# puzzlepaint/camera_calibration

Hardware: NVIDIA H100
Metric: LM iterations/sec (higher is better)
Workload: dtype f64

## Files before the change

camera_calibration_b200/csrc/ba_dense.cu:

```cuda

#include <algorithm>
#include <cstdio>

#include "ba_kernels.h"
#include "ba_tile.cuh"

namespace b200ba {

namespace {

constexpr int BM = 128;
constexpr int LDT = BM + 4;
__host__ __device__ constexpr int gemm_threads(int bn) { return 4 * (bn / 32) * 32; }
constexpr size_t gemm_smem(int bn, int bk, int stages) {
  return static_cast<size_t>(stages) * bk * (LDT + bn + 4) * sizeof(double);
}

__device__ __forceinline__ void cp_async16(void* smem, const void* gmem, int src_bytes) {
  const unsigned s = static_cast<unsigned>(__cvta_generic_to_shared(smem));
  asm volatile("cp.async.cg.shared.global [%0], [%1], 16, %2;\n" ::"r"(s), "l"(gmem), "r"(src_bytes));
}
__device__ __forceinline__ void cp_async8(void* smem, const void* gmem, int src_bytes) {
  const unsigned s = static_cast<unsigned>(__cvta_generic_to_shared(smem));
  asm volatile("cp.async.ca.shared.global [%0], [%1], 8, %2;\n" ::"r"(s), "l"(gmem), "r"(src_bytes));
// ... 23 lines not shown

  __device__ __forceinline__ void init(const double* __restrict__ X, int64_t ldx, int rows, int i0, bool al) {
    aligned = al;
    int i;
    if (al) {
      kk0 = threadIdx.x / CH;
      const int ch = threadIdx.x % CH;
      i = i0 + 2 * ch;
      off0 = kk0 * LD + 2 * ch;
      bytes = (i + 1 < rows) ? 16 : ((i < rows) ? 8 : 0);
    } else {
      kk0 = threadIdx.x / W;
      const int ii = threadIdx.x % W;
      i = i0 + ii;
      off0 = kk0 * LD + ii;
      bytes = (i < rows) ? 8 : 0;
    }
    src = X + static_cast<int64_t>(kk0) * ldx + min(i, max(rows - 1, 0));
  }
  __device__ __forceinline__ void issue(double* dst, int k0, int K, const double* __restrict__ X, int64_t ldx) {
    const double* p = src;
    if (aligned) {
#pragma unroll
      for (int q = 0; q < Q16; ++q) {
        const int nb = (k0 + kk0 + q * KS16 < K) ? bytes : 0;
        cp_async16(dst + off0 + q * KS16 * LD, nb ? p : X, nb);
        p += KS16 * ldx;
      }
    } else {
#pragma unroll
      for (int q = 0; q < Q8; ++q) {
        const int nb = (k0 + kk0 + q * KS8 < K) ? bytes : 0;
        cp_async8(dst + off0 + q * KS8 * LD, nb ? p : X, nb);
        p += KS8 * ldx;
      }
    }
    src += BK * ldx;
  }
};

}

template <bool LOWER, int EPI, int BN_, int BK, int STAGES>
__global__ void __launch_bounds__(gemm_threads(BN_), 2) dgemm_nt_kernel(GemmArgs g) {
  constexpr int THREADS = gemm_threads(BN_);
  constexpr int LDB = BN_ + 4;
  extern __shared__ __align__(16) double smem_d[];
  double* As = smem_d;
  double* Bs = smem_d + static_cast<size_t>(STAGES) * BK * LDT;
  const int warp = threadIdx.x >> 5, lane = threadIdx.x & 31;
  const int wm = (warp & 3) * 32, wn = (warp >> 2) * 32;
  const int lr = lane >> 2, lc = lane & 3;
  constexpr int Q = BM / BN_;
  const int tiles_m = (g.M + BM - 1) / BM, tiles_n = (g.N + BN_ - 1) / BN_;
  const int64_t n_tiles = LOWER ? g.n_tiles_lower : static_cast<int64_t>(tiles_m) * tiles_n;
  const int t_full = min(tiles_m, tiles_n / Q);
  const int64_t tri = static_cast<int64_t>(Q) * t_full * (t_full + 1) / 2;
  for (int64_t tile = blockIdx.x; tile < n_tiles; tile += gridDim.x) {
    int tm, tn;
    if (LOWER) {
      if (tile < tri) {
        tm = static_cast<int>((sqrt(8.0 * static_cast<double>(tile) / Q + 1.0) - 1.0) * 0.5);
        while (static_cast<int64_t>(Q) * tm * (tm + 1) / 2 > tile) --tm;
        while (static_cast<int64_t>(Q) * (tm + 1) * (tm + 2) / 2 <= tile) ++tm;
        tn = static_cast<int>(tile - static_cast<int64_t>(Q) * tm * (tm + 1) / 2);
      } else {
        const int64_t rest = tile - tri;
        tm = t_full + static_cast<int>(rest / tiles_n);
        tn = static_cast<int>(rest - static_cast<int64_t>(tm - t_full) * tiles_n);
      }
    } else {
      tm = static_cast<int>(tile / tiles_n);
      tn = static_cast<int>(tile - static_cast<int64_t>(tm) * tiles_n);
    }
    const int m0 = tm * BM, n0 = tn * BN_;
    if (EPI == 2) {
      const int blk = (g.col_base + n0) / g.map.nb;
      if (blk % g.map.ranks != g.rank) continue;
    }
    __syncthreads();

    double acc[4][4][2];
#pragma unroll
    for (int i = 0; i < 4; ++i)
#pragma unroll
      for (int j = 0; j < 4; ++j) acc[i][j][0] = acc[i][j][1] = 0.0;

    const int nk = (g.K + BK - 1) / BK;
    TileLoader<BK, BM, THREADS> la;
    TileLoader<BK, BN_, THREADS> lb;
    la.init(g.A, g.lda, g.M, m0, g.a_aligned);
    lb.init(g.B, g.ldb, g.N, n0, g.b_aligned);
#pragma unroll
    for (int s = 0; s < STAGES - 1; ++s) {
      if (s < nk) {
        la.issue(As + s * BK * LDT, s * BK, g.K, g.A, g.lda);
        lb.issue(Bs + s * BK * LDB, s * BK, g.K, g.B, g.ldb);
      }
      cp_async_commit();
    }
    for (int kt = 0; kt < nk; ++kt) {
      cp_async_wait<STAGES - 2>();
      __syncthreads();
      {
        const int nt = kt + STAGES - 1;
        if (nt < nk) {
          const int s = nt % STAGES;
          la.issue(As + s * BK * LDT, nt * BK, g.K, g.A, g.lda);
          lb.issue(Bs + s * BK * LDB, nt * BK, g.K, g.B, g.ldb);
        }
        cp_async_commit();
      }
      const double* a_s = As + (kt % STAGES) * BK * LDT;
      const double* b_s = Bs + (kt % STAGES) * BK * LDB;
#pragma unroll
      for (int ks = 0; ks < BK / 4; ++ks) {
        double af[4];
        const double* ap = a_s + (ks * 4 + lc) * LDT + wm + lr;
        const double* bp = b_s + (ks * 4 + lc) * LDB + wn + lr;
#pragma unroll
        for (int i = 0; i < 4; ++i) af[i] = ap[8 * i];
#pragma unroll
        for (int j = 0; j < 4; ++j) {
          const double bf = bp[8 * j];
#pragma unroll
          for (int b = 0; b < 2; ++b)
            dmma1684(acc[2 * b][j][0], acc[2 * b][j][1], acc[2 * b + 1][j][0], acc[2 * b + 1][j][1], af[2 * b],
                     af[2 * b + 1], bf);
        }
      }
    }
    cp_async_wait<0>();

    int rowidx[4];
    bool rowok[4];
#pragma unroll
    for (int i = 0; i < 4; ++i) {
      const int m = m0 + wm + 8 * i + lr;
      rowok[i] = m < g.M;
      rowidx[i] = (EPI == 1) ? (rowok[i] ? __ldg(g.cols + m) : 0) : m;
    }
#pragma unroll
    for (int j = 0; j < 4; ++j) {
#pragma unroll
      for (int e = 0; e < 2; ++e) {
        const int n = n0 + wn + 8 * j + 2 * lc + e;
        if (n >= g.N) continue;
        double* ccol = (EPI == 0) ? (g.C + static_cast<int64_t>(n) * g.ldc)
                                  : (EPI == 1 ? (g.C + g.map.col_offset(__ldg(g.cols + n)))
                                              : (g.C + g.map.col_offset(g.col_base + n) + g.col_base));
        double old[4];
        bool ok[4];
#pragma unroll
        for (int i = 0; i < 4; ++i) {
          ok[i] = rowok[i] && !(LOWER && (m0 + wm + 8 * i + lr) < n);
          old[i] = (ok[i] && g.beta != 0.0) ? ccol[rowidx[i]] : 0.0;
        }
#pragma unroll
        for (int i = 0; i < 4; ++i)
          if (ok[i]) ccol[rowidx[i]] = fma(g.beta, old[i], g.alpha * acc[i][j][e]);
      }
    }
  }
}

int launch_dgemm_nt(const GemmArgs& g_in, bool lower, bool scatter, cudaStream_t s, bool one_tile_per_cta) {
  if (g_in.M <= 0 || g_in.N <= 0) return 0;
  constexpr int BN = 64, BK = 16, STAGES = 4;
  constexpr int T = gemm_threads(BN);
  constexpr int smem = static_cast<int>(gemm_smem(BN, BK, STAGES));
  static bool configured_dev[64] = {};
  static int sm_count[64] = {};
  int dev = 0;
  cudaGetDevice(&dev);
  bool& configured = configured_dev[dev & 63];
  if (!configured) {
    cudaFuncSetAttribute(dgemm_nt_kernel<true, 0, BN, BK, STAGES>, cudaFuncAttributeMaxDynamicSharedMemorySize, smem);
    cudaFuncSetAttribute(dgemm_nt_kernel<false, 0, BN, BK, STAGES>, cudaFuncAttributeMaxDynamicSharedMemorySize, smem);
    cudaFuncSetAttribute(dgemm_nt_kernel<true, 1, BN, BK, STAGES>, cudaFuncAttributeMaxDynamicSharedMemorySize, smem);
    cudaFuncSetAttribute(dgemm_nt_kernel<true, 2, BN, BK, STAGES>, cudaFuncAttributeMaxDynamicSharedMemorySize, smem);
    cudaDeviceGetAttribute(&sm_count[dev & 63], cudaDevAttrMultiProcessorCount, dev);
    configured = true;
  }
  GemmArgs g = g_in;
  constexpr int q = BM / BN;
  const int64_t tm = (g.M + BM - 1) / BM, tn = (g.N + BN - 1) / BN;
  const bool tri_enum = lower || scatter || g.owned_only;
  int64_t n_tiles;
  if (tri_enum) {
    const int64_t t_full = std::min<int64_t>(tm, tn / q);
    n_tiles = q * t_full * (t_full + 1) / 2 + (tm - t_full) * tn;
    g.n_tiles_lower = n_tiles;
  } else {
    n_tiles = tm * tn;
  }
  const int cap = std::max(1, sm_count[dev & 63] * 2);
  const unsigned grid = static_cast<unsigned>(one_tile_per_cta ? n_tiles : std::min<int64_t>(n_tiles, cap));
  if (g.owned_only)
    dgemm_nt_kernel<true, 2, BN, BK, STAGES><<<grid, T, smem, s>>>(g);
  else if (scatter)
    dgemm_nt_kernel<true, 1, BN, BK, STAGES><<<grid, T, smem, s>>>(g);
  else if (tri_enum)
    dgemm_nt_kernel<true, 0, BN, BK, STAGES><<<grid, T, smem, s>>>(g);
  else
    dgemm_nt_kernel<false, 0, BN, BK, STAGES><<<grid, T, smem, s>>>(g);
  return cudaGetLastError() == cudaSuccess ? 0 : 1;
}

constexpr int PT = 128;

struct TileDeviceExec {
  tile::Thread t;
  template <class F>
  __host__ __device__ __forceinline__ void run(F f) {
#if defined(__CUDA_ARCH__)
    f(t, static_cast<int>(threadIdx.x));
    __syncthreads();
#else
    (void)f;
#endif
  }
};
__global__ void __launch_bounds__(tile::THREADS, 1)
    potrf_trinv_tile_kernel(const double* __restrict__ Ain, int64_t lda_in, int n, double* __restrict__ Lout, int64_t lda_out,
                            double* __restrict__ Linv, int* __restrict__ info) {
  extern __shared__ __align__(16) unsigned char tile_smem[];
  tile::Shared& sh = *reinterpret_cast<tile::Shared*>(tile_smem);
  TileDeviceExec ex;
  tile::potrf_trinv_program(ex, sh, Ain, lda_in, n, Lout, lda_out, Linv, static_cast<int>(blockIdx.x), info);
}
int launch_potrf_trinv_tile(const double* Ain, int64_t lda_in, int n, double* Lout, int64_t lda_out, double* Linv, int* info,
                            cudaStream_t s) {
  static bool configured_dev[64] = {};
  int dev = 0;
  cudaGetDevice(&dev);
  if (!configured_dev[dev & 63]) {
    cudaFuncSetAttribute(potrf_trinv_tile_kernel, cudaFuncAttributeMaxDynamicSharedMemorySize, static_cast<int>(sizeof(tile::Shared)));
    configured_dev[dev & 63] = true;
  }
  potrf_trinv_tile_kernel<<<tile::CTAS, tile::THREADS, sizeof(tile::Shared), s>>>(Ain, lda_in, n, Lout, lda_out, Linv, info);
  return cudaGetLastError() == cudaSuccess ? 0 : 1;
}

__global__ void add_diagonal_map_kernel(int n, double* S, DenseMap map, double lambda) {
  const int c = blockIdx.x * blockDim.x + threadIdx.x;
  if (c < n) S[map.col_offset(c) + c] += lambda;
}
void launch_add_diagonal_map(int n, double* S, const DenseMap& map, double lambda, cudaStream_t s) {
  if (n > 0) add_diagonal_map_kernel<<<(n + 255) / 256, 256, 0, s>>>(n, S, map, lambda);
}

// ... 369 lines not shown
```

camera_calibration_b200/csrc/ba_host.cu:

```cuda

#include <cublas_v2.h>
#include <cusolverDn.h>
#include <dlfcn.h>

#include <algorithm>
#include <cmath>
#include <cstdarg>
#include <cstdio>
#include <cstring>
#include <limits>
#include <string>
#include <vector>

#include "ba_kernels.h"

using namespace b200ba;

namespace {

std::string g_create_error;

struct NcclUniqueId {
  char internal[128];
};
// ... 56 lines not shown
  std::string error;

  std::vector<b200ba_camera> cams_host;
  ProblemDev pb{};
  int n_cameras = 0, n_imagesets = 0, n_points = 0;
  int64_t n_obs = 0;
  int uniform_model = -1;
  int64_t n_control_total = 0, n_param_total = 0, intr_total = 0, tan_total = 0;
  uint32_t *d_obs_imageset = nullptr, *d_obs_camera = nullptr, *d_obs_point = nullptr;
  float2* d_obs_xy = nullptr;

  StateDev st[2]{};
  int cur = 0;
  double2* d_last_projection = nullptr;
  bool have_state = false;
  StateDev snap{};
  double2* d_snap_lp = nullptr;
  bool have_snapshot = false;

  Layout L{};
  bool have_layout = false;
  ObsOut out{};
  ObsOut out_trial{};
  SystemDev sys{};
  double *d_W = nullptr, *d_S = nullptr, *d_Linv = nullptr, *d_v = nullptr, *d_y = nullptr, *d_x = nullptr;
  double trace_H = 0;
  int64_t reduce_count = 0;
  double* d_potrf_work = nullptr;
  int potrf_lwork = 0;
  int *d_info = nullptr, *d_fail = nullptr;
  std::vector<uint32_t> perm;
  uint32_t* d_perm = nullptr;
  double2* d_lp_stage = nullptr;
  uint32_t* d_straggler_list = nullptr;
  int* d_straggler_count = nullptr;
  double *d_partial = nullptr, *d_scal = nullptr;
  double* d_rot = nullptr;
  double* h_scal = nullptr;
  int* h_flags = nullptr;

  std::vector<uint32_t> h_obs_imageset, h_obs_camera, h_obs_point;
  std::vector<float> h_obs_xy;
  int group_blocks_n = 0;
  int n_groups = 0;
  std::vector<int> group_start;
  std::vector<int> group_count;
  int* d_group_of_block = nullptr;
  int* d_group_blocks = nullptr;
  uint8_t* d_flags = nullptr;
  int* d_cols = nullptr;
  int* d_count = nullptr;
  int* h_count = nullptr;
  double* d_Wc = nullptr;
  double* d_P = nullptr;
  size_t wc_stride = 0, p_stride = 0;
  cudaEvent_t ev_syrk[2] = {nullptr, nullptr}, ev_scatter[2] = {nullptr, nullptr}, ev_s_ready = nullptr;
  double* d_u = nullptr;
  bool use_grouped = false;
  double* capture_S = nullptr;
  double* capture_rhs = nullptr;
  std::vector<int32_t> lm_events;
  std::vector<double> grp_sums;
  int force_grouped = -1;

  ReportDev rep{};
  double2* d_rep_stage = nullptr;
  bool have_report = false;
  std::vector<int64_t> img_cam_groups;
  int* d_img_group_off = nullptr;
  uint32_t* d_img_group_obs = nullptr;
  bool have_images = false;

  void* comm = nullptr;
  int rank = 0, n_ranks = 1;

  bool own_dense = true;
  DenseCtx dn;
  int dense_planned_ranks = 0, dense_planned_n = -1;
  int dense_nb = 0;
  cudaStream_t panel_stream = nullptr;
  cudaStream_t aux_stream = nullptr;
  int* d_ident_cols = nullptr;
  double* d_gemv_partial = nullptr;

  b200ba_timings timings{};
  struct Pending {
    int phase;
    cudaEvent_t a, b;
    bool own_a = true;
  };
  std::vector<Pending> pending;
  std::vector<cudaEvent_t> event_pool;
};

namespace {

#define CUDA_TRY(h, expr)                                                                      \
  do {                                                                                         \
    cudaError_t _e = (expr);                                                                   \
    if (_e != cudaSuccess) {                                                                   \
      (h)->error = std::string(#expr) + ": " + cudaGetErrorString(_e);                         \
      return 1;                                                                                \
    }                                                                                          \
  } while (0)
#define CUBLAS_TRY(h, expr)                                                                    \
  do {                                                                                         \
// ... 127 lines not shown
  const cudaError_t ce = cudaStreamSynchronize(h->stream);
  if (rc == 0 && ce == cudaSuccess) cudaMemcpy(h->grp_sums.data(), d, n * sizeof(double), cudaMemcpyDeviceToHost);
  cudaFree(d);
  if (rc != 0 || ce != cudaSuccess) {
    h->error = "all-reduce of the group centroids failed";
    return 1;
  }
  return 0;
}

int build_groups(b200ba_handle* h, bool allocate) {
  const Layout& L = h->L;
  const int nb = L.nblocks;
  int gb = (L.bs == 3) ? 96 : 48;
  if (const char* e = getenv("B200BA_GROUP_BLOCKS")) gb = std::max(1, atoi(e));
  h->group_blocks_n = gb;
  std::vector<int> order(nb);
  for (int i = 0; i < nb; ++i) order[i] = i;
  if (L.eliminate_points && nb > 0) {
    const double* sx = h->grp_sums.data();
    const double* sy = sx + nb;
    const double* cnt = sy + nb;
    const double qx = std::max(1.0, h->cams_host[0].width / 64.0), qy = std::max(1.0, h->cams_host[0].height / 64.0);
    std::vector<uint32_t> zkey(nb, 0);
    for (int p = 0; p < nb; ++p) {
      if (cnt[p] <= 0) continue;
      uint32_t ux = static_cast<uint32_t>(std::min(1023.0, std::max(0.0, sx[p] / cnt[p] / qx)));
      uint32_t uy = static_cast<uint32_t>(std::min(1023.0, std::max(0.0, sy[p] / cnt[p] / qy)));
      uint32_t z = 0;
      for (int b = 0; b < 10; ++b) z |= ((ux >> b) & 1u) << (2 * b) | ((uy >> b) & 1u) << (2 * b + 1);
      zkey[p] = z;
    }
    std::stable_sort(order.begin(), order.end(), [&](int a, int b) { return zkey[a] < zkey[b]; });
  }
  h->n_groups = (nb + gb - 1) / gb;
  h->group_start.assign(h->n_groups + 1, 0);
  std::vector<int> gob(std::max(1, nb), 0);
  for (int g = 0; g < h->n_groups; ++g) {
    h->group_start[g] = g * gb;
    for (int i = g * gb; i < std::min(nb, (g + 1) * gb); ++i) gob[order[i]] = g;
  }
  h->group_start[h->n_groups] = nb;
  h->group_count.assign(std::max(1, h->n_groups), 0);
  if (allocate) {
    if (dev_alloc(h, &h->d_group_of_block, std::max(1, nb))) return 1;
    if (dev_alloc(h, &h->d_group_blocks, std::max(1, nb))) return 1;
    if (dev_alloc(h, &h->d_flags, static_cast<size_t>(std::max(1, h->n_groups)) * std::max(1, L.nd))) return 1;
    if (dev_alloc(h, &h->d_cols, static_cast<size_t>(std::max(1, h->n_groups)) * std::max(1, L.nd))) return 1;
    if (dev_alloc(h, &h->d_count, std::max(1, h->n_groups))) return 1;
    if (h->h_count) cudaFreeHost(h->h_count);
    CUDA_TRY(h, cudaMallocHost(reinterpret_cast<void**>(&h->h_count), std::max(1, h->n_groups) * sizeof(int)));
    h->wc_stride = static_cast<size_t>(gb) * L.bs * (std::max(1, L.nd) + 1);
    h->p_stride = static_cast<size_t>(std::max(1, L.nd)) * std::max(1, L.nd);
    if (dev_alloc(h, &h->d_Wc, 2 * h->wc_stride)) return 1;
    if (!h->own_dense && dev_alloc(h, &h->d_P, 2 * h->p_stride)) return 1;
    for (int i = 0; i < 2; ++i) {
      if (!h->ev_syrk[i]) CUDA_TRY(h, cudaEventCreateWithFlags(&h->ev_syrk[i], cudaEventDisableTiming));
      if (!h->ev_scatter[i]) CUDA_TRY(h, cudaEventCreateWithFlags(&h->ev_scatter[i], cudaEventDisableTiming));
    }
    if (!h->ev_s_ready) CUDA_TRY(h, cudaEventCreateWithFlags(&h->ev_s_ready, cudaEventDisableTiming));
    if (dev_alloc(h, &h->d_u, std::max(1, L.nbd))) return 1;
  }
  CUDA_TRY(h, cudaMemcpy(h->d_group_of_block, gob.data(), std::max(1, nb) * sizeof(int), cudaMemcpyHostToDevice));
  if (nb > 0) CUDA_TRY(h, cudaMemcpy(h->d_group_blocks, order.data(), nb * sizeof(int), cudaMemcpyHostToDevice));
  return 0;
}

int nccl_bcast_cb(double* buf, size_t count, int root, cudaStream_t s, void* user) {
  b200ba_handle* h = static_cast<b200ba_handle*>(user);
  const int rc = g_nccl.Broadcast(buf, buf, count, kNcclDouble, root, h->comm, s);
  if (rc != 0) {
    h->error = std::string("ncclBroadcast: ") + (g_nccl.GetErrorString ? g_nccl.GetErrorString(rc) : "error");
    return 1;
  }
  return 0;
}

cudaError_t dense_create(DenseCtx* d, bool own_streams) {
  cudaError_t e = cudaSuccess;
  if (own_streams) {
    int lo = 0, hi = 0;
    cudaDeviceGetStreamPriorityRange(&lo, &hi);
    e = cudaStreamCreateWithFlags(&d->s_main, cudaStreamNonBlocking);
    if (e == cudaSuccess) e = cudaStreamCreateWithPriority(&d->s_panel, cudaStreamNonBlocking, hi);
    if (e == cudaSuccess) e = cudaStreamCreateWithPriority(&d->s_aux, cudaStreamNonBlocking, hi);
  }
  for (cudaEvent_t* ev : {&d->ev_ready[0], &d->ev_ready[1], &d->ev_main[0], &d->ev_main[1], &d->ev_half2[0],
                          &d->ev_half2[1], &d->ev_misc})
    if (e == cudaSuccess && !*ev) e = cudaEventCreateWithFlags(ev, cudaEventDisableTiming);
  return e;
}
void dense_release(DenseCtx* d, bool own_streams) {
  for (cudaEvent_t ev : {d->ev_ready[0], d->ev_ready[1], d->ev_main[0], d->ev_main[1], d->ev_half2[0], d->ev_half2[1],
                         d->ev_misc})
    if (ev) cudaEventDestroy(ev);
  if (own_streams)
    for (cudaStream_t s : {d->s_main, d->s_panel, d->s_aux})
      if (s) cudaStreamDestroy(s);
}

int plan_dense(b200ba_handle* h) {
  if (!h->own_dense || !h->have_layout) return 0;
  const int nd = h->L.nd;
  if (h->dense_planned_n == nd && h->dense_planned_ranks == h->n_ranks) return 0;
  DenseCtx& d = h->dn;
  const int nb = h->dense_nb > 0 ? h->dense_nb : (h->n_ranks == 1 ? 512 : 256);
  dense_plan(&d, nd, nb, h->rank, h->n_ranks);
// ... 397 lines not shown
      CUBLAS_TRY(h, cublasDgemv(h->cublas, CUBLAS_OP_T, L.nd, L.nbd, &one, h->sys.B, L.nd, h->d_x + L.nbd, 1, &zero,
                                h->d_y, 1));
    launch_block_backsub2(L.bs, L.nblocks, h->d_Linv, h->d_u, h->d_y, h->d_x, h->stream);
    h->timings.kernel_launches += 1;
  } else {
    ScopedPhase ph(h, PH_SCHUR);
    CUDA_TRY(h, cudaMemcpyAsync(h->d_y, h->d_v, L.nbd * sizeof(double), cudaMemcpyDeviceToDevice, h->stream));
    if (L.nbd > 0 && L.nd > 0)
      CUBLAS_TRY(h, cublasDgemv(h->cublas, CUBLAS_OP_T, L.nd, L.nbd, &minus_one, h->d_W, L.nd, h->d_x + L.nbd, 1, &one,
                                h->d_y, 1));
    launch_schur_backsub(L.bs, L.nblocks, h->d_Linv, h->d_y, h->d_x, h->stream);
    h->timings.kernel_launches += 1;
  }
  CUDA_TRY(h, cudaMemcpyAsync(h->h_flags, h->d_info, sizeof(int), cudaMemcpyDeviceToHost, h->stream));
  CUDA_TRY(h, cudaMemcpyAsync(h->h_flags + 1, h->d_fail, sizeof(int), cudaMemcpyDeviceToHost, h->stream));
  if (sync_stream(h)) return 1;
  *spd = (h->h_flags[0] == 0 && h->h_flags[1] == 0) ? 1 : 0;
  return 0;
}

int solve_system_own(b200ba_handle* h, double lambda, int* spd) {
  const Layout& L = h->L;
  DenseCtx& d = h->dn;
  const int nd = L.nd, R = h->n_ranks;
  {
    ScopedPhase ph(h, PH_SCHUR);
    CUDA_TRY(h, cudaMemsetAsync(h->d_fail, 0, sizeof(int), h->stream));
    CUDA_TRY(h, cudaMemsetAsync(h->d_info, 0, sizeof(int), h->stream));
    launch_schur_blocks(L.bs, L.nblocks, h->sys.Dblk, h->sys.bp, lambda, h->d_Linv, h->d_v, h->d_fail, h->stream);
    CUDA_TRY(h, cudaEventRecord(h->ev_s_ready, h->stream));
    CUDA_TRY(h, cudaStreamWaitEvent(h->side_stream, h->ev_s_ready, 0));
    if (nd > 0) {
      if (R == 1) {
        CUDA_TRY(h, cudaMemcpy2DAsync(h->d_S, d.map.ld * sizeof(double), h->sys.C, static_cast<size_t>(nd) * sizeof(double),
                                      static_cast<size_t>(nd) * sizeof(double), nd, cudaMemcpyDeviceToDevice, h->side_stream));
      } else {
        for (int j = 0; j < d.nblk; ++j) {
          const int c0 = j * d.NB, w = std::min(d.NB, nd - c0);
          CUDA_TRY(h, cudaMemcpy2DAsync(h->d_S + d.map.col_offset(c0), d.map.ld * sizeof(double),
                                        h->sys.C + static_cast<size_t>(c0) * nd, static_cast<size_t>(nd) * sizeof(double),
                                        static_cast<size_t>(nd) * sizeof(double), w, cudaMemcpyDeviceToDevice, h->side_stream));
        }
      }
    }
    CUDA_TRY(h, cudaEventRecord(h->ev_s_ready, h->side_stream));
    launch_block_solve_t(L.bs, L.nblocks, h->d_Linv, h->d_v, h->d_u, h->stream);
    h->timings.kernel_launches += 2;
    bool joined = false;
    auto join_copy = [&]() {
      if (!joined) cudaStreamWaitEvent(h->stream, h->ev_s_ready, 0);
      joined = true;
    };
    if (h->use_grouped) {
      int it = 0;
      for (int g = h->rank; g < h->n_groups; g += R) {
        const int nblk = h->group_start[g + 1] - h->group_start[g];
        const int kg = nblk * L.bs, mg = h->group_count[g];
        if (mg == 0 || kg == 0) continue;
        const int ldw = (mg + 1) / 2 * 2;
        double* Wc = h->d_Wc + (it & 1) * h->wc_stride;
        const int* cols = h->d_cols + static_cast<size_t>(g) * nd;
        launch_gather_scale(L.bs, nblk, nd, mg, ldw, h->sys.B, h->d_Linv, h->d_group_blocks + h->group_start[g], cols, Wc,
                            h->stream);
        join_copy();
        GemmArgs ga{};
        ga.M = ga.N = mg;
        ga.K = kg;
        ga.A = ga.B = Wc;
        ga.lda = ga.ldb = ldw;
        ga.C = h->d_S;
        ga.alpha = -1.0;
        ga.beta = 1.0;
        ga.a_aligned = ga.b_aligned = gemm_operand_aligned(Wc, ldw);
        ga.cols = cols;
        ga.map = d.map;
        if (launch_dgemm_nt(ga, true, true, h->stream)) {
          h->error = "dgemm_nt (contraction) launch failed";
          return 1;
        }
        h->timings.contraction_flops += static_cast<double>(mg) * mg * kg;
        h->timings.kernel_launches += 2;
        ++it;
      }
    } else if (L.nbd > 0 && nd > 0) {
      const int p0 = static_cast<int>(static_cast<int64_t>(L.nblocks) * h->rank / R);
      const int p1 = static_cast<int>(static_cast<int64_t>(L.nblocks) * (h->rank + 1) / R);
      const int k_rows = L.bs * (p1 - p0);
      launch_schur_scale_rows(L.bs, L.nblocks, nd, h->sys.B, h->d_Linv, h->d_W, h->stream);
      h->timings.kernel_launches += 1;
      if (k_rows > 0) {
        const double* Wr = h->d_W + static_cast<size_t>(L.bs) * p0 * nd;
        join_copy();
        GemmArgs ga{};
        ga.M = ga.N = nd;
        ga.K = k_rows;
        ga.A = ga.B = Wr;
        ga.lda = ga.ldb = nd;
        ga.C = h->d_S;
        ga.ldc = d.map.ld;
        ga.alpha = -1.0;
        ga.beta = 1.0;
        ga.a_aligned = ga.b_aligned = gemm_operand_aligned(Wr, nd);
        ga.cols = h->d_ident_cols;
        ga.map = d.map;
        if (launch_dgemm_nt(ga, true, R > 1, h->stream)) {
          h->error = "dgemm_nt (contraction) launch failed";
          return 1;
        }
        h->timings.contraction_flops += static_cast<double>(nd) * nd * k_rows;
        h->timings.kernel_launches += 1;
      }
    }
    join_copy();
    if (h->rank == 0) launch_add_diagonal_map(nd, h->d_S, d.map, lambda, h->stream);
    CUDA_TRY(h, cudaMemcpyAsync(h->d_x + L.nbd, h->sys.bd, nd * sizeof(double), cudaMemcpyDeviceToDevice, h->stream));
    if (L.nbd > 0 && nd > 0) launch_gemv_t(L.nbd, nd, nd, h->sys.B, h->d_u, -1.0, h->d_x + L.nbd, h->d_gemv_partial, h->stream);
    h->timings.kernel_launches += 4;
  }
  if (h->capture_S && capture_reduced_system(h)) return 1;
  if (R > 1 && nd > 0) {
    ScopedPhase ph(h, PH_ALLREDUCE);
    const int rc = g_nccl.ReduceScatter(h->d_S, h->d_S + static_cast<size_t>(h->rank) * d.chunk, static_cast<size_t>(d.chunk),
                                        kNcclDouble, kNcclSum, h->comm, h->stream);
    if (rc != 0) {
      h->error = std::string("ncclReduceScatter: ") + (g_nccl.GetErrorString ? g_nccl.GetErrorString(rc) : "error");
      return 1;
    }
  }
  {
    ScopedPhase ph(h, PH_FACTOR);
    if (dense_factor(&d)) {
      if (h->error.empty()) h->error = "dense_factor: launch failed";
      return 1;
    }
    h->timings.factor_flops += static_cast<double>(nd) * nd * nd / 3.0;
// ... 11 lines not shown
      h->error = "dense_solve: launch failed";
      return 1;
    }
    h->timings.kernel_launches += 4 * d.ntiles;
  }
  {
    ScopedPhase ph(h, PH_SCHUR);
    if (L.nbd > 0 && nd > 0)
      launch_gemv_n(L.nbd, nd, nd, h->sys.B, h->d_x + L.nbd, h->d_y, h->stream);
    else if (L.nbd > 0)
      CUDA_TRY(h, cudaMemsetAsync(h->d_y, 0, L.nbd * sizeof(double), h->stream));
    launch_block_backsub2(L.bs, L.nblocks, h->d_Linv, h->d_u, h->d_y, h->d_x, h->stream);
    h->timings.kernel_launches += 1;
  }
  CUDA_TRY(h, cudaMemcpyAsync(h->h_flags, h->d_info, sizeof(int), cudaMemcpyDeviceToHost, h->stream));
  CUDA_TRY(h, cudaMemcpyAsync(h->h_flags + 1, h->d_fail, sizeof(int), cudaMemcpyDeviceToHost, h->stream));
  if (sync_stream(h)) return 1;
  *spd = (h->h_flags[0] == 0 && h->h_flags[1] == 0) ? 1 : 0;
  return 0;
}

int check_ready(b200ba_handle* h, const b200ba_options* opt) {
  if (!h) return 1;
  if (!opt) {
    h->error = "options are NULL";
    return 2;
  }
  if (!h->have_state) {
    h->error = "no state: call b200ba_set_state first";
    return 2;
  }
  CUDA_TRY(h, cudaSetDevice(h->device));
  return make_layout(h, opt);
}

void free_handle_buffers(b200ba_handle* h) {
  auto F = [](auto*& p) {
    if (p) cudaFree(p);
    p = nullptr;
  };
  F(h->d_obs_imageset); F(h->d_obs_camera); F(h->d_obs_point); F(h->d_obs_xy);
  for (int i = 0; i < 2; ++i) {
    F(h->st[i].points); F(h->st[i].rig_tr_global); F(h->st[i].camera_tr_rig); F(h->st[i].intrinsics);
    F(h->st[i].image_tr_global); F(h->st[i].tangents);
  }
  F(h->d_last_projection);
  F(h->snap.points); F(h->snap.rig_tr_global); F(h->snap.camera_tr_rig); F(h->snap.intrinsics); F(h->d_snap_lp);
  h->have_snapshot = false;
  F(h->out.residual); F(h->out.cost); F(h->out.jac); F(h->out.cjac); F(h->out.cell); F(h->out.has_jac); F(h->out.evals);
  F(h->out_trial.residual); F(h->out_trial.cost);
  F(h->sys.base); F(h->d_W); F(h->d_S); F(h->d_Linv); F(h->d_v); F(h->d_y); F(h->d_x); F(h->d_potrf_work);
  F(h->d_info); F(h->d_fail); F(h->d_straggler_list); F(h->d_straggler_count); F(h->d_perm); F(h->d_lp_stage);
  F(h->d_group_of_block); F(h->d_group_blocks); F(h->d_flags); F(h->d_cols); F(h->d_count); F(h->d_Wc); F(h->d_P); F(h->d_u);
  if (h->h_count) cudaFreeHost(h->h_count);
  h->h_count = nullptr;
  F(h->d_partial); F(h->d_scal); F(h->d_rot);
  F(h->rep.err); F(h->rep.mag); F(h->rep.cam_off); F(h->rep.cell_off); F(h->rep.cell_order); F(h->rep.Q);
  F(h->rep.partial); F(h->rep.select_hist); F(h->rep.hist); F(h->rep.kl); F(h->rep.cams); F(h->d_rep_stage);
  h->have_report = false;
  F(h->d_img_group_off); F(h->d_img_group_obs);
  h->have_images = false;
  F(h->dn.Lpack); F(h->dn.tmp); F(h->dn.d_panel_off); F(h->dn.d_panel_h); F(h->d_ident_cols); F(h->d_gemv_partial);
  h->dn.S = nullptr;
  h->dense_planned_n = -1;
  if (h->h_scal) cudaFreeHost(h->h_scal);
  if (h->h_flags) cudaFreeHost(h->h_flags);
  h->h_scal = nullptr;
  h->h_flags = nullptr;
}

int setup_report(b200ba_handle* h) {
  if (h->have_report) return 0;
  const int64_t n = h->n_obs;
  const int nc = h->n_cameras;
  constexpr int kCells = kReportBiasCells * kReportBiasCells;
  std::vector<int64_t> cam_off(nc + 1, 0);
  for (int64_t o = 0; o < n; ++o) ++cam_off[h->h_obs_camera[o] + 1];
  for (int c = 0; c < nc; ++c) cam_off[c + 1] += cam_off[c];
  std::vector<uint32_t> key(n);
  std::vector<int> cell_off(static_cast<size_t>(nc) * kCells + 1, 0);
  for (int64_t o = 0; o < n; ++o) {
    const uint32_t cam = h->h_obs_camera[o];
    const b200ba_camera& c = h->cams_host[cam];
    const double step_u = static_cast<double>(c.calibration_max_x - c.calibration_min_x) / kReportBiasCells + 1e-7;
    const double step_v = static_cast<double>(c.calibration_max_y - c.calibration_min_y) / kReportBiasCells + 1e-7;
    const float dx = h->h_obs_xy[2 * o] - static_cast<float>(c.calibration_min_x);
    const float dy = h->h_obs_xy[2 * o + 1] - static_cast<float>(c.calibration_min_y);
    const int cx = std::min(kReportBiasCells - 1, std::max(0, static_cast<int>(dx / step_u)));
    const int cy = std::min(kReportBiasCells - 1, std::max(0, static_cast<int>(dy / step_v)));
    key[o] = cam * kCells + cy * kReportBiasCells + cx;
    ++cell_off[key[o] + 1];
  }
  for (size_t k = 0; k + 1 < cell_off.size(); ++k) cell_off[k + 1] += cell_off[k];
  std::vector<uint32_t> pos(n), order(n);
  for (int64_t i = 0; i < n; ++i) pos[h->perm[i]] = static_cast<uint32_t>(i);
  {
    std::vector<int> fill(cell_off.begin(), cell_off.end() - 1);
    for (int64_t o = 0; o < n; ++o) order[fill[key[o]]++] = pos[o];
  }
  double Q[64], q_sum = 0;
  for (int y = 0; y < 8; ++y)
    for (int x = 0; x < 8; ++x) {
      const double dx = (2.5 / (0.5 * 8)) * (0.5 * 8 - (x + 0.5));
      const double dy = (2.5 / (0.5 * 8)) * (0.5 * 8 - (y + 0.5));
      const double p = std::exp(-0.5 * (dx * dx + dy * dy));
      Q[y * 8 + x] = p;
      q_sum += p;
    }
// ... 2804 lines not shown
```

camera_calibration_b200/csrc/ba_kernels.h:

```cpp
#pragma once
#include <vector>

#include "ba_common.h"

namespace b200ba {

void launch_prepare_state(const ProblemDev& pb, const Layout& L, const StateDev& st, int64_t n_control_total,
                          cudaStream_t s);
void launch_residual_jacobian(int uniform_model, bool jac, const ProblemDev& pb, const Layout& L,
                              const StateDev& st, double2* last_projection, const ObsOut& out, double huber,
                              uint32_t* straggler_list, int* straggler_count, cudaStream_t s,
                              cudaEvent_t main_done = nullptr);
void launch_straggler_pass(int uniform_model, bool jac, const ProblemDev& pb, const Layout& L, const StateDev& st,
                           double2* last_projection, const ObsOut& out, double huber, uint32_t* straggler_list,
                           int* straggler_count, cudaStream_t s);
void launch_accumulate_list(const ProblemDev& pb, const Layout& L, const StateDev& st, const ObsOut& out,
                            const SystemDev& sys, double huber, const uint32_t* list, const int* count, cudaStream_t s);
void launch_expand_jacobian(const ProblemDev& pb, const Layout& L, const StateDev& st, const ObsOut& out, double* jac,
                            cudaStream_t s);
void set_main_eval_budget(int budget);
void launch_accumulate_scatter(const ProblemDev& pb, const Layout& L, const StateDev& st, const ObsOut& out,
                               const SystemDev& sys, double huber, cudaStream_t s);
void launch_accumulate_cells(const ProblemDev& pb, const Layout& L, const StateDev& st, const ObsOut& out,
                             const SystemDev& sys, double huber, cudaStream_t s);
// ... 56 lines not shown
                             cudaStream_t s);
void launch_intersect_features(int d, int64_t n_lists, int64_t max_list, const int64_t* off, float2* xy, float bound,
                               uint8_t* keep, float2* centres, int* n_centres, unsigned long long* counts,
                               cudaStream_t s);
constexpr int kSynthTile = 16;
constexpr int kSynthMaxVerts = 4;
struct SynthParams {
  int w, h, tiles_x, tiles_y, words, n_poly;
  float fx, fy, cx, cy;
  int pattern_w, pattern_h, squares_x, squares_y, num_tags;
  float page_w, page_h, start_x, start_y, end_x, end_y;
  int4 tags[B200BA_PATTERN_MAX_TAGS];
};
void launch_render_pattern(const SynthParams& p, int n_img, const float2* verts, const int8_t* nv, const float* poses,
                           const uint8_t* pattern, double2* proj, int4* range, uint32_t* bits, uint8_t* images,
                           cudaStream_t s);
struct RefineParams {
  int w, h;
  int half;
  int n_samples, n_match;
  int type;
  int num_star_segments, squares_x, squares_y, num_tags;
  int4 tags[B200BA_PATTERN_MAX_TAGS];
};
void launch_refine_features(const RefineParams& p, int64_t n, const b200ba_feature_prediction* pred,
                            const uint8_t* images, const float2* samples, float2* xy, float* cost, int* status,
                            cudaStream_t s);
void launch_generic_block_inverse(int bs, int nb, int nd, const double* D, const double* B, const double* b1,
                                  double* DinvB, double* Dinvb, cudaStream_t s);
void launch_symmetrize(int n, double* M, cudaStream_t s);
void launch_dirfit_tangents(int G, const double* grid, double* tan, cudaStream_t s);
void launch_dirfit(bool jac, int gw, int64_t n, const double* gp, const double* dirs, const double* grid,
                   const double* tan, double* H, double* b, int dof, double* cost, double* cost_sum, cudaStream_t s);
void launch_dirfit_update(int G, const double* grid, const double* x, double* out, cudaStream_t s);
void launch_permute_double2(int64_t n, const uint32_t* perm, const double2* src, double2* dst, bool scatter,
                            cudaStream_t s);


void launch_mask_fixed(const Layout& L, const SystemDev& sys, const FixedRanges& fr, double unit, cudaStream_t s);
void launch_nice_orientation(const ProblemDev& pb, const StateDev& st, int n_cameras, double* rot, cudaStream_t s);

struct DenseMap {
  int nb;
  int ranks;
  int blocks_per_rank;
  int64_t ld;
  __host__ __device__ __forceinline__ int slot(int block) const { return (block % ranks) * blocks_per_rank + block / ranks; }
  __host__ __device__ __forceinline__ int64_t col_offset(int c) const {
    const int b = c / nb;
    return (static_cast<int64_t>(slot(b)) * nb + (c - b * nb)) * ld;
  }
};

struct GemmArgs {
  int M, N, K;
  const double* A;
  int64_t lda;
  const double* B;
  int64_t ldb;
  double* C;
  int64_t ldc;
  double alpha, beta;
  bool a_aligned, b_aligned;
  const int* cols;
  DenseMap map;
  int64_t n_tiles_lower;
  bool owned_only;
  int rank, col_base;
};
inline bool gemm_operand_aligned(const double* p, int64_t ld) {
  return (reinterpret_cast<uintptr_t>(p) % 16 == 0) && (ld % 2 == 0);
}
int launch_dgemm_nt(const GemmArgs& g, bool lower, bool scatter, cudaStream_t s, bool one_tile_per_cta = false);

int gemv_t_partial_size(int rows, int cols);
void launch_gemv_t(int rows, int cols, int64_t ld, const double* B, const double* u, double alpha, double* y, double* partial,
                   cudaStream_t s);
void launch_gemv_n(int rows, int cols, int64_t ld, const double* B, const double* x, double* t, cudaStream_t s);
void launch_add_diagonal_map(int n, double* S, const DenseMap& map, double lambda, cudaStream_t s);

struct DenseCtx {
  int n = 0, NB = 256, nblk = 0, ntiles = 0;
  int rank = 0, ranks = 1;
  DenseMap map{};
  int64_t chunk = 0;
  std::vector<int64_t> panel_off;
  std::vector<int> panel_h;
  double* S = nullptr;
  double* Lpack = nullptr;
  double* tmp = nullptr;
  int64_t* d_panel_off = nullptr;
  int* d_panel_h = nullptr;
  int* info = nullptr;
  cudaStream_t s_main = nullptr, s_panel = nullptr, s_aux = nullptr;
  cudaEvent_t ev_ready[2] = {nullptr, nullptr}, ev_main[2] = {nullptr, nullptr}, ev_half2[2] = {nullptr, nullptr}, ev_misc = nullptr;
  int (*bcast)(double* buf, size_t count, int root, cudaStream_t s, void* user) = nullptr;
  void* user = nullptr;
};
int dense_plan(DenseCtx* d, int n, int nb, int rank, int ranks);
int dense_factor(DenseCtx* d);
int dense_solve(DenseCtx* d, double* b);

}
```

Before: 23.35.

## Batch per-group Schur contractions into one grouped lower-triangular DGEMM launch

Replaces the per-group loop, which launched gather_scale and a scatter DGEMM for each group through double-buffered Wc, with gathering every group into one contiguous Wc buffer. A single grouped DGEMM (EPI=3) then runs over all groups, using a device-side table and a binary search to map each tile to its group. The aim is to remove per-group launch overhead and the serialization between small GEMMs, so that tiles from all groups fill the SMs together. In exchange, results are written with atomicAdd instead of read-modify-write, which makes floating-point summation order nondeterministic. It also adds a host-to-device table copy and a larger Wc allocation.

```diff
diff --git a/camera_calibration_b200/csrc/ba_dense.cu b/camera_calibration_b200/csrc/ba_dense.cu
--- a/camera_calibration_b200/csrc/ba_dense.cu
+++ b/camera_calibration_b200/csrc/ba_dense.cu
@@ -99,11 +99,37 @@
   const int wm = (warp & 3) * 32, wn = (warp >> 2) * 32;
   const int lr = lane >> 2, lc = lane & 3;
   constexpr int Q = BM / BN_;
-  const int tiles_m = (g.M + BM - 1) / BM, tiles_n = (g.N + BN_ - 1) / BN_;
+  int M = g.M, N = g.N, K = g.K;
+  const double* A = g.A;
+  const double* Bop = g.B;
+  int64_t lda = g.lda, ldb = g.ldb;
+  const int* cols = g.cols;
+  bool a_al = g.a_aligned, b_al = g.b_aligned;
+  int tiles_m = (M + BM - 1) / BM, tiles_n = (N + BN_ - 1) / BN_;
+  int t_full = min(tiles_m, tiles_n / Q);
+  int64_t tri = static_cast<int64_t>(Q) * t_full * (t_full + 1) / 2;
   const int64_t n_tiles = LOWER ? g.n_tiles_lower : static_cast<int64_t>(tiles_m) * tiles_n;
-  const int t_full = min(tiles_m, tiles_n / Q);
-  const int64_t tri = static_cast<int64_t>(Q) * t_full * (t_full + 1) / 2;
-  for (int64_t tile = blockIdx.x; tile < n_tiles; tile += gridDim.x) {
+  for (int64_t tile_g = blockIdx.x; tile_g < n_tiles; tile_g += gridDim.x) {
+    int64_t tile = tile_g;
+    if (EPI == 3) {
+      int lo = 0, hi = g.n_groups - 1;
+      while (lo < hi) {
+        const int mid = (lo + hi + 1) >> 1;
+        if (g.groups[mid].tile0 <= tile_g) lo = mid; else hi = mid - 1;
+      }
+      const ContractGroup cg = g.groups[lo];
+      tile = tile_g - cg.tile0;
+      M = N = cg.m;
+      K = cg.k;
+      A = Bop = g.A + cg.w_off;
+      lda = ldb = cg.ld;
+      cols = g.cols + cg.cols_off;
+      a_al = b_al = cg.aligned;
+      tiles_m = (M + BM - 1) / BM;
+      tiles_n = (N + BN_ - 1) / BN_;
+      t_full = min(tiles_m, tiles_n / Q);
+      tri = static_cast<int64_t>(Q) * t_full * (t_full + 1) / 2;
+    }
     int tm, tn;
     if (LOWER) {
       if (tile < tri) {
@@ -133,16 +159,16 @@
 #pragma unroll
       for (int j = 0; j < 4; ++j) acc[i][j][0] = acc[i][j][1] = 0.0;
 
-    const int nk = (g.K + BK - 1) / BK;
+    const int nk = (K + BK - 1) / BK;
     TileLoader<BK, BM, THREADS> la;
     TileLoader<BK, BN_, THREADS> lb;
-    la.init(g.A, g.lda, g.M, m0, g.a_aligned);
-    lb.init(g.B, g.ldb, g.N, n0, g.b_aligned);
+    la.init(A, lda, M, m0, a_al);
+    lb.init(Bop, ldb, N, n0, b_al);
 #pragma unroll
     for (int s = 0; s < STAGES - 1; ++s) {
       if (s < nk) {
-        la.issue(As + s * BK * LDT, s * BK, g.K, g.A, g.lda);
-        lb.issue(Bs + s * BK * LDB, s * BK, g.K, g.B, g.ldb);
+        la.issue(As + s * BK * LDT, s * BK, K, A, lda);
+        lb.issue(Bs + s * BK * LDB, s * BK, K, Bop, ldb);
       }
       cp_async_commit();
     }
@@ -153,8 +179,8 @@
         const int nt = kt + STAGES - 1;
         if (nt < nk) {
           const int s = nt % STAGES;
-          la.issue(As + s * BK * LDT, nt * BK, g.K, g.A, g.lda);
-          lb.issue(Bs + s * BK * LDB, nt * BK, g.K, g.B, g.ldb);
+          la.issue(As + s * BK * LDT, nt * BK, K, A, lda);
+          lb.issue(Bs + s * BK * LDB, nt * BK, K, Bop, ldb);
         }
         cp_async_commit();
       }
@@ -179,36 +205,49 @@
     }
     cp_async_wait<0>();
 
+    constexpr bool SCATTER = EPI == 1 || EPI == 3;
     int rowidx[4];
     bool rowok[4];
 #pragma unroll
     for (int i = 0; i < 4; ++i) {
       const int m = m0 + wm + 8 * i + lr;
-      rowok[i] = m < g.M;
-      rowidx[i] = (EPI == 1) ? (rowok[i] ? __ldg(g.cols + m) : 0) : m;
+      rowok[i] = m < M;
+      rowidx[i] = SCATTER ? (rowok[i] ? __ldg(cols + m) : 0) : m;
     }
 #pragma unroll
     for (int j = 0; j < 4; ++j) {
 #pragma unroll
       for (int e = 0; e < 2; ++e) {
         const int n = n0 + wn + 8 * j + 2 * lc + e;
-        if (n >= g.N) continue;
+        if (n >= N) continue;
         double* ccol = (EPI == 0) ? (g.C + static_cast<int64_t>(n) * g.ldc)
-                                  : (EPI == 1 ? (g.C + g.map.col_offset(__ldg(g.cols + n)))
-                                              : (g.C + g.map.col_offset(g.col_base + n) + g.col_base));
+                                  : (SCATTER ? (g.C + g.map.col_offset(__ldg(cols + n)))
+                                             : (g.C + g.map.col_offset(g.col_base + n) + g.col_base));
+        bool ok[4];
+#pragma unroll
+        for (int i = 0; i < 4; ++i) ok[i] = rowok[i] && !(LOWER && (m0 + wm + 8 * i + lr) < n);
+        if (EPI == 3) {
+#pragma unroll
+          for (int i = 0; i < 4; ++i)
+            if (ok[i]) atomicAdd(ccol + rowidx[i], g.alpha * acc[i][j][e]);
+          continue;
+        }
         double old[4];
-        bool ok[4];
-#pragma unroll
-        for (int i = 0; i < 4; ++i) {
-          ok[i] = rowok[i] && !(LOWER && (m0 + wm + 8 * i + lr) < n);
-          old[i] = (ok[i] && g.beta != 0.0) ? ccol[rowidx[i]] : 0.0;
-        }
+#pragma unroll
+        for (int i = 0; i < 4; ++i) old[i] = (ok[i] && g.beta != 0.0) ? ccol[rowidx[i]] : 0.0;
 #pragma unroll
         for (int i = 0; i < 4; ++i)
           if (ok[i]) ccol[rowidx[i]] = fma(g.beta, old[i], g.alpha * acc[i][j][e]);
       }
     }
   }
+}
+
+int64_t dgemm_lower_tiles(int M, int N) {
+  constexpr int BN = 64, q = BM / BN;
+  const int64_t tm = (M + BM - 1) / BM, tn = (N + BN - 1) / BN;
+  const int64_t t_full = std::min<int64_t>(tm, tn / q);
+  return q * t_full * (t_full + 1) / 2 + (tm - t_full) * tn;
 }
 
 int launch_dgemm_nt(const GemmArgs& g_in, bool lower, bool scatter, cudaStream_t s, bool one_tile_per_cta) {
@@ -226,24 +265,27 @@
     cudaFuncSetAttribute(dgemm_nt_kernel<false, 0, BN, BK, STAGES>, cudaFuncAttributeMaxDynamicSharedMemorySize, smem);
     cudaFuncSetAttribute(dgemm_nt_kernel<true, 1, BN, BK, STAGES>, cudaFuncAttributeMaxDynamicSharedMemorySize, smem);
     cudaFuncSetAttribute(dgemm_nt_kernel<true, 2, BN, BK, STAGES>, cudaFuncAttributeMaxDynamicSharedMemorySize, smem);
+    cudaFuncSetAttribute(dgemm_nt_kernel<true, 3, BN, BK, STAGES>, cudaFuncAttributeMaxDynamicSharedMemorySize, smem);
     cudaDeviceGetAttribute(&sm_count[dev & 63], cudaDevAttrMultiProcessorCount, dev);
     configured = true;
   }
   GemmArgs g = g_in;
-  constexpr int q = BM / BN;
-  const int64_t tm = (g.M + BM - 1) / BM, tn = (g.N + BN - 1) / BN;
   const bool tri_enum = lower || scatter || g.owned_only;
   int64_t n_tiles;
-  if (tri_enum) {
-    const int64_t t_full = std::min<int64_t>(tm, tn / q);
-    n_tiles = q * t_full * (t_full + 1) / 2 + (tm - t_full) * tn;
+  if (g.groups) {
+    n_tiles = g.n_tiles_lower;
+    if (n_tiles <= 0 || g.n_groups <= 0) return 0;
+  } else if (tri_enum) {
+    n_tiles = dgemm_lower_tiles(g.M, g.N);
     g.n_tiles_lower = n_tiles;
   } else {
-    n_tiles = tm * tn;
+    n_tiles = static_cast<int64_t>((g.M + BM - 1) / BM) * ((g.N + BN - 1) / BN);
   }
   const int cap = std::max(1, sm_count[dev & 63] * 2);
   const unsigned grid = static_cast<unsigned>(one_tile_per_cta ? n_tiles : std::min<int64_t>(n_tiles, cap));
-  if (g.owned_only)
+  if (g.groups)
+    dgemm_nt_kernel<true, 3, BN, BK, STAGES><<<grid, T, smem, s>>>(g);
+  else if (g.owned_only)
     dgemm_nt_kernel<true, 2, BN, BK, STAGES><<<grid, T, smem, s>>>(g);
   else if (scatter)
     dgemm_nt_kernel<true, 1, BN, BK, STAGES><<<grid, T, smem, s>>>(g);
diff --git a/camera_calibration_b200/csrc/ba_host.cu b/camera_calibration_b200/csrc/ba_host.cu
--- a/camera_calibration_b200/csrc/ba_host.cu
+++ b/camera_calibration_b200/csrc/ba_host.cu
@@ -132,6 +132,8 @@
   int* d_count = nullptr;
   int* h_count = nullptr;
   double* d_Wc = nullptr;
+  ContractGroup* h_contract = nullptr;
+  ContractGroup* d_contract = nullptr;
   double* d_P = nullptr;
   size_t wc_stride = 0, p_stride = 0;
   cudaEvent_t ev_syrk[2] = {nullptr, nullptr}, ev_scatter[2] = {nullptr, nullptr}, ev_s_ready = nullptr;
@@ -365,7 +367,11 @@
     CUDA_TRY(h, cudaMallocHost(reinterpret_cast<void**>(&h->h_count), std::max(1, h->n_groups) * sizeof(int)));
     h->wc_stride = static_cast<size_t>(gb) * L.bs * (std::max(1, L.nd) + 1);
     h->p_stride = static_cast<size_t>(std::max(1, L.nd)) * std::max(1, L.nd);
-    if (dev_alloc(h, &h->d_Wc, 2 * h->wc_stride)) return 1;
+    const size_t wc_n = h->own_dense ? static_cast<size_t>(std::max(1, L.nbd)) * (std::max(1, L.nd) + 1) : 2 * h->wc_stride;
+    if (dev_alloc(h, &h->d_Wc, wc_n)) return 1;
+    if (dev_alloc(h, &h->d_contract, std::max(1, h->n_groups))) return 1;
+    if (h->h_contract) cudaFreeHost(h->h_contract);
+    CUDA_TRY(h, cudaMallocHost(reinterpret_cast<void**>(&h->h_contract), std::max(1, h->n_groups) * sizeof(ContractGroup)));
     if (!h->own_dense && dev_alloc(h, &h->d_P, 2 * h->p_stride)) return 1;
     for (int i = 0; i < 2; ++i) {
       if (!h->ev_syrk[i]) CUDA_TRY(h, cudaEventCreateWithFlags(&h->ev_syrk[i], cudaEventDisableTiming));
@@ -869,35 +875,48 @@
       joined = true;
     };
     if (h->use_grouped) {
-      int it = 0;
+      int n_tab = 0;
+      int64_t w_off = 0, tiles = 0;
       for (int g = h->rank; g < h->n_groups; g += R) {
         const int nblk = h->group_start[g + 1] - h->group_start[g];
         const int kg = nblk * L.bs, mg = h->group_count[g];
         if (mg == 0 || kg == 0) continue;
         const int ldw = (mg + 1) / 2 * 2;
-        double* Wc = h->d_Wc + (it & 1) * h->wc_stride;
-        const int* cols = h->d_cols + static_cast<size_t>(g) * nd;
-        launch_gather_scale(L.bs, nblk, nd, mg, ldw, h->sys.B, h->d_Linv, h->d_group_blocks + h->group_start[g], cols, Wc,
-                            h->stream);
+        ContractGroup& cg = h->h_contract[n_tab++];
+        cg.w_off = w_off;
+        cg.cols_off = static_cast<int64_t>(g) * nd;
+        cg.tile0 = tiles;
+        cg.m = mg;
+        cg.k = kg;
+        cg.ld = ldw;
+        cg.aligned = gemm_operand_aligned(h->d_Wc + w_off, ldw);
+        launch_gather_scale(L.bs, nblk, nd, mg, ldw, h->sys.B, h->d_Linv, h->d_group_blocks + h->group_start[g],
+                            h->d_cols + cg.cols_off, h->d_Wc + w_off, h->stream);
+        w_off += static_cast<int64_t>(kg) * ldw;
+        tiles += dgemm_lower_tiles(mg, mg);
+        h->timings.contraction_flops += static_cast<double>(mg) * mg * kg;
+        h->timings.kernel_launches += 1;
+      }
+      if (n_tab > 0) {
+        CUDA_TRY(h, cudaMemcpyAsync(h->d_contract, h->h_contract, n_tab * sizeof(ContractGroup), cudaMemcpyHostToDevice,
+                                    h->stream));
         join_copy();
         GemmArgs ga{};
-        ga.M = ga.N = mg;
-        ga.K = kg;
-        ga.A = ga.B = Wc;
-        ga.lda = ga.ldb = ldw;
+        ga.A = h->d_Wc;
         ga.C = h->d_S;
         ga.alpha = -1.0;
         ga.beta = 1.0;
-        ga.a_aligned = ga.b_aligned = gemm_operand_aligned(Wc, ldw);
-        ga.cols = cols;
+        ga.cols = h->d_cols;
         ga.map = d.map;
+        ga.groups = h->d_contract;
+        ga.n_groups = n_tab;
+        ga.n_tiles_lower = tiles;
+        ga.M = ga.N = ga.K = 1;
         if (launch_dgemm_nt(ga, true, true, h->stream)) {
           h->error = "dgemm_nt (contraction) launch failed";
           return 1;
         }
-        h->timings.contraction_flops += static_cast<double>(mg) * mg * kg;
-        h->timings.kernel_launches += 2;
-        ++it;
+        h->timings.kernel_launches += 1;
       }
     } else if (L.nbd > 0 && nd > 0) {
       const int p0 = static_cast<int>(static_cast<int64_t>(L.nblocks) * h->rank / R);
@@ -1015,8 +1034,11 @@
   F(h->sys.base); F(h->d_W); F(h->d_S); F(h->d_Linv); F(h->d_v); F(h->d_y); F(h->d_x); F(h->d_potrf_work);
   F(h->d_info); F(h->d_fail); F(h->d_straggler_list); F(h->d_straggler_count); F(h->d_perm); F(h->d_lp_stage);
   F(h->d_group_of_block); F(h->d_group_blocks); F(h->d_flags); F(h->d_cols); F(h->d_count); F(h->d_Wc); F(h->d_P); F(h->d_u);
+  F(h->d_contract);
   if (h->h_count) cudaFreeHost(h->h_count);
   h->h_count = nullptr;
+  if (h->h_contract) cudaFreeHost(h->h_contract);
+  h->h_contract = nullptr;
   F(h->d_partial); F(h->d_scal); F(h->d_rot);
   F(h->rep.err); F(h->rep.mag); F(h->rep.cam_off); F(h->rep.cell_off); F(h->rep.cell_order); F(h->rep.Q);
   F(h->rep.partial); F(h->rep.select_hist); F(h->rep.hist); F(h->rep.kl); F(h->rep.cams); F(h->d_rep_stage);
diff --git a/camera_calibration_b200/csrc/ba_kernels.h b/camera_calibration_b200/csrc/ba_kernels.h
--- a/camera_calibration_b200/csrc/ba_kernels.h
+++ b/camera_calibration_b200/csrc/ba_kernels.h
@@ -132,6 +132,12 @@
   }
 };
 
+struct ContractGroup {
+  int64_t w_off, cols_off, tile0;
+  int m, k, ld;
+  bool aligned;
+};
+
 struct GemmArgs {
   int M, N, K;
   const double* A;
@@ -147,11 +153,14 @@
   int64_t n_tiles_lower;
   bool owned_only;
   int rank, col_base;
+  const ContractGroup* groups;
+  int n_groups;
 };
 inline bool gemm_operand_aligned(const double* p, int64_t ld) {
   return (reinterpret_cast<uintptr_t>(p) % 16 == 0) && (ld % 2 == 0);
 }
 int launch_dgemm_nt(const GemmArgs& g, bool lower, bool scatter, cudaStream_t s, bool one_tile_per_cta = false);
+int64_t dgemm_lower_tiles(int M, int N);
 
 int gemv_t_partial_size(int rows, int cols);
 void launch_gemv_t(int rows, int cols, int64_t ld, const double* B, const double* u, double alpha, double* y, double* partial,
```

Result: faster. 24.27, median of 6 (+3.9%).
